# argumentcomputer/multi-stark

Hardware: AMD Instinct MI355X
Metric: prove_trace_rows_per_sec (higher is better)
Workload: dtype u64; 1 GPU; U32-add + byte-table lookup (benches/multi_stark.rs), 2^20 additions per proof, bench_config(): log_blowup 2, 100 queries, 10+10 PoW bits, GoldilocksBlake3Config; witness (traces + claims, 64-bit words) in pinned host memory at step start: upload, from_stage_1 on the device and read-back inside the timed region; the library narrows byte-valued traces on host threads INSIDE the step before they cro; rows_per_proof=1048832, proof_bytes=1100053, parallelism=single GPU

## Files before the change

### multi-stark_amd/csrc/b3_quad.h

```cpp
#pragma once
#include "b3_dev.h"

namespace msamd {

namespace b3q {
constexpr unsigned char S[7][16] = {{0, 1, 2, 3, 4, 5, 6, 7, 8, 9, 10, 11, 12, 13, 14, 15},
                                    {2, 6, 3, 10, 7, 0, 4, 13, 1, 11, 12, 5, 9, 14, 15, 8},
                                    {3, 4, 10, 12, 13, 2, 7, 14, 6, 5, 9, 0, 11, 15, 8, 1},
                                    {10, 7, 12, 9, 14, 3, 13, 15, 4, 0, 11, 2, 5, 8, 1, 6},
                                    {12, 13, 9, 11, 15, 10, 14, 8, 7, 2, 5, 3, 0, 1, 6, 4},
                                    {9, 14, 11, 5, 8, 12, 15, 1, 13, 3, 0, 10, 2, 6, 4, 7},
                                    {11, 15, 5, 0, 1, 9, 8, 6, 14, 10, 2, 12, 3, 4, 7, 13}};
constexpr u32 packed(int r, int k) {
  u32 p = 0;
  for (int c = 0; c < 4; c++) {
    int pos = (k < 2 ? 2 * c + k : 8 + 2 * c + (k - 2));
    p |= (u32)S[r][pos] << (4 * c);
  }
  return p;
}
__device__ __forceinline__ u32 qperm(u32 x, int ctrl) {
#if !defined(__HIP_DEVICE_COMPILE__)
  return x;
#else
// ... 39 lines not shown
#pragma unroll
  for (int r = 0; r < 7; r++) {
    B3Q_G(mw[r][0], mw[r][1])
    b = b3q::qperm(b, 0x39);
    cc = b3q::qperm(cc, 0x4E);
    d = b3q::qperm(d, 0x93);
    B3Q_G(mw[r][2], mw[r][3])
    b = b3q::qperm(b, 0x93);
    cc = b3q::qperm(cc, 0x4E);
    d = b3q::qperm(d, 0x39);
  }
  h_lo = a ^ cc;
  h_hi = b ^ d;
}

__device__ __forceinline__ void b3_quad_compress_cv(const u32* msg, u32 block_len, u32 flags, u32& lo, u32& hi) {
  const u32 c = threadIdx.x & 3;
  const u32 sh4 = 4 * c;
  u32 mw[7][4];
#pragma unroll
  for (int r = 0; r < 7; r++) {
#pragma unroll
    for (int k = 0; k < 4; k++) mw[r][k] = msg[(b3q::packed(r, k) >> sh4) & 15u];
  }
  u32 a = lo, b = hi;
  u32 cc = c == 0 ? B3_IV0 : c == 1 ? B3_IV1 : c == 2 ? B3_IV2 : B3_IV3;
  u32 d = c == 2 ? block_len : c == 3 ? flags : 0u;
#pragma unroll
  for (int r = 0; r < 7; r++) {
    B3Q_G(mw[r][0], mw[r][1])
    b = b3q::qperm(b, 0x39);
    cc = b3q::qperm(cc, 0x4E);
    d = b3q::qperm(d, 0x93);
    B3Q_G(mw[r][2], mw[r][3])
    b = b3q::qperm(b, 0x93);
    cc = b3q::qperm(cc, 0x4E);
    d = b3q::qperm(d, 0x39);
  }
  lo = a ^ cc;
  hi = b ^ d;
}

// ... 9 lines not shown
```

### multi-stark_amd/csrc/hash.hip

```cpp
#include <algorithm>
#include <cstdlib>
#include <cstring>

#include "b3_dev.h"
#include "b3_quad.h"
#include "outer_dev.h"
#include "challenge_dev.h"
#include "fri_dev.h"
#include "msamd.h"
#include "tree_dev.h"

namespace msamd {

namespace {

struct RowIter {
  const MatRef* g;
  size_t H, row;
  unsigned mi;
  u32 c;
  const u64* cur;
  u32 w;
  size_t stride;
  __device__ __forceinline__ void init() {
// ... 511 lines not shown
    }
  }
  if (CH) {
    challenger_round<1024>(cs, sh, p.fc.pow_bits);
    if (t < 8) {
      p.fc.state[t] = cs.st[t];
      p.fc.rec->root[t] = sh[t];
    }
    if (t == 0) {
      p.fc.rec->witness = cs.wit;
      p.fc.rec->beta = cs.beta;
    }
  }
}

__device__ __forceinline__ u32 stream_byte(const uint8_t* __restrict__ prefix, size_t pl, const u64* __restrict__ words, size_t p) {
  if (p < pl) return prefix[p];
  size_t q = p - pl;
  return (u32)((words[q >> 3] >> (8 * (q & 7))) & 0xff);
}

__global__ __launch_bounds__(256) void chunk_cv_k(const uint8_t* __restrict__ prefix, size_t pl, const u64* __restrict__ words,
                                                  size_t len, size_t nchunks, size_t c0, size_t c1, Digest* out) {
  size_t ch = c0 + blockIdx.x * size_t(blockDim.x) + threadIdx.x;
  if (ch >= c1) return;
  size_t off = ch * 1024;
  size_t clen = len - off < 1024 ? len - off : 1024;
  u32 nblocks = clen == 0 ? 1 : (u32)((clen + 63) / 64);
  u32 cv[8];
  b3_iv(cv);
  const bool single = nchunks == 1;
  for (u32 b = 0; b < nblocks; b++) {
    u32 m[16];
    size_t boff = off + size_t(b) * 64;
    u32 bl = (u32)(clen - size_t(b) * 64 < 64 ? clen - size_t(b) * 64 : 64);
    if (bl == 64 && boff >= pl) {
      size_t q = boff - pl;
      const u64* w = words + (q >> 3);
      unsigned s = (unsigned)(q & 7) * 8;
      u64 cur = w[0];
#pragma unroll
      for (int k = 0; k < 8; k++) {
        u64 x;
        if (s == 0) {
          x = cur;
          if (k < 7) cur = w[k + 1];
        } else {
          u64 nxt = w[k + 1];
          x = (cur >> s) | (nxt << (64 - s));
          cur = nxt;
        }
        m[2 * k] = (u32)x;
        m[2 * k + 1] = (u32)(x >> 32);
      }
    } else {
#pragma unroll
      for (int i = 0; i < 16; i++) {
        u32 wv = 0;
        for (int k = 0; k < 4; k++) {
          u32 idx = 4 * i + k;
          u32 byte = idx < bl ? stream_byte(prefix, pl, words, boff + idx) : 0;
          wv |= byte << (8 * k);
        }
        m[i] = wv;
      }
    }
    u32 flags = (b == 0 ? B3_CHUNK_START : 0) | (b == nblocks - 1 ? (B3_CHUNK_END | (single ? B3_ROOT : 0)) : 0);
    b3_compress(cv, m, ch, bl, flags);
  }
  store_digest(out + ch, cv);
}

__global__ __launch_bounds__(64) void chunk_cv_prefix_k(const uint8_t* __restrict__ prefix, size_t pl, const u64* __restrict__ words,
                                                        size_t len, size_t nchunks, size_t c0, Digest* out) {
  __shared__ u32 sh[256];
  const size_t ch = c0 + blockIdx.x;
  const size_t off = ch * 1024;
  const size_t clen = len - off < 1024 ? len - off : 1024;
  for (u32 i = threadIdx.x; i < 256; i += 64) {
    u32 wv = 0;
#pragma unroll
    for (u32 k = 0; k < 4; k++) {
      const u32 idx = 4 * i + k;
      const u32 byte = idx < clen ? stream_byte(prefix, pl, words, off + idx) : 0;
      wv |= byte << (8 * k);
    }
    sh[i] = wv;
  }
  __syncthreads();
  if (threadIdx.x != 0) return;
  const u32 nblocks = clen == 0 ? 1 : (u32)((clen + 63) / 64);
  u32 cv[8];
  b3_iv(cv);
  const bool single = nchunks == 1;
  for (u32 b = 0; b < nblocks; b++) {
    u32 m[16];
#pragma unroll
    for (int i = 0; i < 16; i++) m[i] = sh[16 * b + i];
    const u32 bl = (u32)(clen - size_t(b) * 64 < 64 ? clen - size_t(b) * 64 : 64);
    const u32 flags = (b == 0 ? B3_CHUNK_START : 0) | (b == nblocks - 1 ? (B3_CHUNK_END | (single ? B3_ROOT : 0)) : 0);
    b3_compress(cv, m, ch, bl, flags);
  }
  store_digest(out + ch, cv);
}

__global__ __launch_bounds__(256) void cv_level_k(const Digest* __restrict__ prev, Digest* __restrict__ next, size_t n_prev,
                                                  u32 root_flag) {
  size_t n_next = (n_prev + 1) / 2;
  size_t i = blockIdx.x * size_t(blockDim.x) + threadIdx.x;
  if (i >= n_next) return;
  u32 l[8];
  load_digest(prev + 2 * i, l);
  if (2 * i + 1 < n_prev) {
    u32 r[8], o[8];
    load_digest(prev + 2 * i + 1, r);
    parent_cv(l, r, root_flag, o);
    store_digest(next + i, o);
  } else {
    store_digest(next + i, l);
  }
}

__global__ __launch_bounds__(1024) void cv_tail_k(const Digest* __restrict__ prev, Digest* __restrict__ out, u32 n, Digest* __restrict__ sib_out = nullptr) {
  __shared__ __attribute__((aligned(16))) u32 sh[2048 * 8];
  const u32 t = threadIdx.x;
  for (u32 i = t; i < n; i += 1024) {
    u32 d[8];
    load_digest(prev + i, d);
    lds_store_digest(sh, i, d);
  }
  __syncthreads();
  const u32 quad = t >> 2, c = t & 3;
  while (n > 1) {
    const u32 nn = (n + 1) / 2;
    const u32 flags = B3_PARENT | (n == 2 ? (u32)B3_ROOT : 0u);
    if (sib_out) {
      if (t < 8) reinterpret_cast<u32*>(sib_out)[t] = sh[8 + t];
      sib_out++;
    }
    u32 lo[4], hi[4];
#pragma unroll
    for (int ps = 0; ps < 4; ps++) {
      const u32 q = quad + 256 * ps;
      if (q < nn) {
        if (2 * q + 1 < n) {
          b3_quad_compress_iv<false>(sh + 16 * q, 64, flags, lo[ps], hi[ps]);
        } else {
          lo[ps] = sh[16 * q + c];
          hi[ps] = sh[16 * q + 4 + c];
        }
      }
    }
    __syncthreads();
#pragma unroll
    for (int ps = 0; ps < 4; ps++) {
      const u32 q = quad + 256 * ps;
      if (q < nn) {
        sh[8 * q + c] = lo[ps];
        sh[8 * q + 4 + c] = hi[ps];
      }
    }
    __syncthreads();
    n = nn;
  }
  if (t < 8) reinterpret_cast<u32*>(out)[t] = sh[t];
}

}

void merkle_alloc(Ctx& ctx, DTree& t, size_t maxh) {
  t.layer_off.clear();
  t.layer_len.clear();
  size_t tot = 0;
  for (size_t l = maxh;; l >>= 1) {
    t.layer_off.push_back(tot);
    t.layer_len.push_back(l);
    tot += l;
    if (l == 1) break;
  }
  t.digests = DBuf<Digest>(ctx, tot);
// ... 252 lines not shown
  HIP_CHECK(hipGetLastError());
}

std::vector<Digest> merkle_cap(Ctx& ctx, const DTree& t) {
  size_t cl = t.cap_layer();
  std::vector<Digest> cap(t.layer_len[cl]);
  ctx.d2h(cap.data(), t.base() + t.layer_off[cl], cap.size() * sizeof(Digest));
  return cap;
}

size_t blake3_num_chunks(size_t prefix_len, size_t nwords) {
  size_t len = prefix_len + 8 * nwords;
  return len == 0 ? 1 : (len + 1023) / 1024;
}

void blake3_chunk_cvs(Ctx& ctx, const uint8_t* d_prefix, size_t prefix_len, const u64* d_words, size_t nwords, size_t c0, size_t c1,
                      Digest* cvs) {
  const size_t len = prefix_len + 8 * nwords, nchunks = blake3_num_chunks(prefix_len, nwords);
  if (c1 > nchunks) c1 = nchunks;
  if (c0 >= c1) return;
  const size_t pc = std::min(c1, (prefix_len + 1023) / 1024);
  if (c0 < pc) {
    hipLaunchKernelGGL(chunk_cv_prefix_k, dim3((unsigned)(pc - c0)), dim3(64), 0, ctx.stream, d_prefix, prefix_len, d_words, len, nchunks, c0, cvs);
    c0 = pc;
  }
  if (c0 < c1)
    hipLaunchKernelGGL(chunk_cv_k, dim3((unsigned)((c1 - c0 + 255) / 256)), dim3(256), 0, ctx.stream, d_prefix, prefix_len, d_words, len,
                       nchunks, c0, c1, cvs);
  HIP_CHECK(hipGetLastError());
}

struct ClaimsRootArgs {
  const uint8_t* prefix;
  const u64* words;
  size_t pl, len;
  const u32* cap;
  u32 cap_off, cap_bytes;
  const Digest* sib[32];
  u32 nchunks;
  Digest* out;
  ChallengeBG* bg;
  u32* state_out;
};
__global__ __launch_bounds__(64) void claims_root_k(ClaimsRootArgs a) {
  __shared__ u32 sh[256];
  __shared__ u32 pm[16];
  const u32 t = threadIdx.x, c = t & 3;
  const u32 clen = a.len < 1024 ? (u32)a.len : 1024u;
  for (u32 i = t; i < 256; i += 64) {
    u32 wv = 0;
#pragma unroll
    for (u32 k = 0; k < 4; k++) {
      const u32 idx = 4 * i + k;
      u32 byte = 0;
      if (idx < clen) {
        if (idx >= a.cap_off && idx - a.cap_off < a.cap_bytes) {
          const u32 q = idx - a.cap_off;
          byte = (a.cap[q >> 2] >> (8 * (q & 3))) & 0xff;
        } else {
          byte = stream_byte(a.prefix, a.pl, a.words, idx);
        }
      }
      wv |= byte << (8 * k);
    }
    sh[i] = wv;
  }
  __syncthreads();
  u32 lo = c == 0 ? B3_IV0 : c == 1 ? B3_IV1 : c == 2 ? B3_IV2 : B3_IV3;
  u32 hi = c == 0 ? B3_IV4 : c == 1 ? B3_IV5 : c == 2 ? B3_IV6 : B3_IV7;
  const u32 nblocks = (clen + 63) / 64;
  for (u32 b = 0; b < nblocks; b++) {
    const u32 bl = clen - 64 * b < 64 ? clen - 64 * b : 64;
    const u32 flags = (b == 0 ? (u32)B3_CHUNK_START : 0u) | (b == nblocks - 1 ? (u32)B3_CHUNK_END : 0u);
    b3_quad_compress_cv(sh + 16 * b, bl, flags, lo, hi);
  }
  for (u32 l = 0; (1u << l) < a.nchunks; l++) {
    if (t < 4) {
      pm[c] = lo;
      pm[4 + c] = hi;
    }
    if (t >= 8 && t < 16) pm[t] = reinterpret_cast<const u32*>(a.sib[l])[t - 8];
    __syncthreads();
    const bool last = (2u << l) >= a.nchunks;
    b3_quad_compress_iv<false>(pm, 64, B3_PARENT | (last ? (u32)B3_ROOT : 0u), lo, hi);
    __syncthreads();
  }
  if (t < 4) {
    u32* o = reinterpret_cast<u32*>(a.out);
    o[c] = lo;
    o[4 + c] = hi;
    pm[c] = lo;
    pm[4 + c] = hi;
  }
  if (a.bg) {
    __syncthreads();
    outer_beta_gamma_step(pm, a.bg, a.state_out);
  }
}

static const Digest* blake3_cv_tree(Ctx& ctx, Digest* cvs, size_t nchunks, DBuf<Digest>& scratch, Digest* out_dev) {
  scratch = DBuf<Digest>(ctx, (nchunks + 1) / 2);
  Digest* cur = cvs;
  Digest* nxt = scratch.p;
  size_t n = nchunks;
  while (n > 1) {
    if (n <= 2048) {
      hipLaunchKernelGGL(cv_tail_k, dim3(1), dim3(1024), 0, ctx.stream, (const Digest*)cur, nxt, (u32)n);
      std::swap(cur, nxt);
      break;
    }
    size_t nn = (n + 1) / 2;
    hipLaunchKernelGGL(cv_level_k, dim3((unsigned)((nn + 255) / 256)), dim3(256), 0, ctx.stream, cur, nxt, n,
                       n == 2 ? (u32)B3_ROOT : 0u);
    std::swap(cur, nxt);
    n = nn;
  }
  HIP_CHECK(hipGetLastError());
  if (out_dev) HIP_CHECK(hipMemcpyAsync(out_dev, cur, sizeof(Digest), hipMemcpyDeviceToDevice, ctx.stream));
  return cur;
}
Digest blake3_from_cvs(Ctx& ctx, Digest* cvs, size_t nchunks) {
  DBuf<Digest> b;
  const Digest* cur = blake3_cv_tree(ctx, cvs, nchunks, b, nullptr);
  Digest out;
  ctx.d2h(&out, cur, sizeof(Digest));
  return out;
}
void blake3_from_cvs_async(Ctx& ctx, Digest* cvs, size_t nchunks, Digest* out_dev) {
  DBuf<Digest> b;
  (void)blake3_cv_tree(ctx, cvs, nchunks, b, out_dev);
}

void blake3_late_chunk0_prepare(Ctx& ctx, const Digest* cvs, size_t nchunks, LateChunk0& lc) {
  if (nchunks < 2 || nchunks > (size_t(1) << 30)) throw std::runtime_error("blake3_late_chunk0: chunk count out of range");
  lc.levels = DBuf<Digest>(ctx, nchunks + 64);
  lc.sib.clear();
  const Digest* cur = cvs;
  Digest* nxt = lc.levels.p;
  size_t n = nchunks;
  while (n > 1) {
    if (n <= 2048) {
      Digest* tail_sib = nxt + 1;
      size_t m = n;
      while (m > 1) {
        lc.sib.push_back(tail_sib++);
        m = (m + 1) / 2;
      }
      hipLaunchKernelGGL(cv_tail_k, dim3(1), dim3(1024), 0, ctx.stream, cur, nxt, (u32)n, nxt + 1);
      break;
    }
    lc.sib.push_back(cur + 1);
    const size_t nn = (n + 1) / 2;
    hipLaunchKernelGGL(cv_level_k, dim3((unsigned)((nn + 255) / 256)), dim3(256), 0, ctx.stream, cur, nxt, n, 0u);
    cur = nxt;
    nxt += nn;
    n = nn;
  }
  HIP_CHECK(hipGetLastError());
  if (lc.sib.size() > 32) throw std::runtime_error("blake3_late_chunk0: too many levels");
}
void blake3_late_chunk0_finish(Ctx& ctx, const uint8_t* d_prefix, size_t prefix_len, const u64* d_words, size_t nwords, const Digest* d_cap,
                               size_t cap_off, size_t ncap, const LateChunk0& lc, size_t nchunks, Digest* out_dev, ChallengeBG* d_bg,
                               u32* d_state12) {
  if (prefix_len > 1024 || cap_off + 32 * ncap > prefix_len) throw std::runtime_error("blake3_late_chunk0: the prefix must lie inside chunk 0");
  ClaimsRootArgs a;
  memset(&a, 0, sizeof(a));
  a.prefix = d_prefix;
  a.words = d_words;
  a.pl = prefix_len;
  a.len = prefix_len + 8 * nwords;
  a.cap = reinterpret_cast<const u32*>(d_cap);
  a.cap_off = (u32)cap_off;
  a.cap_bytes = (u32)(32 * ncap);
  unsigned levels = 0;
  while ((size_t(1) << levels) < nchunks) levels++;
  if (lc.sib.size() != levels) throw std::runtime_error("blake3_late_chunk0: level count mismatch");
  for (unsigned l = 0; l < levels; l++) a.sib[l] = lc.sib[l];
  a.nchunks = (u32)nchunks;
  a.out = out_dev;
  a.bg = d_bg;
  a.state_out = d_state12;
  hipLaunchKernelGGL(claims_root_k, dim3(1), dim3(64), 0, ctx.stream, a);
  HIP_CHECK(hipGetLastError());
}

Digest blake3_device(Ctx& ctx, const uint8_t* d_prefix, size_t prefix_len, const u64* d_words, size_t nwords) {
  const size_t nchunks = blake3_num_chunks(prefix_len, nwords);
  DBuf<Digest> a(ctx, nchunks);
  blake3_chunk_cvs(ctx, d_prefix, prefix_len, d_words, nwords, 0, nchunks, a.p);
  return blake3_from_cvs(ctx, a.p, nchunks);
}

}
```

### multi-stark_amd/csrc/msamd.h

```cpp
#pragma once
#include <hip/hip_runtime.h>

#include <cstdint>
#include <cstring>
#include <map>
#include <mutex>
#include <stdexcept>
#include <string>
#include <vector>

#include "gl_dev.h"

namespace msamd {

#define HIP_CHECK(expr)                                                                                   \
  do {                                                                                                    \
    hipError_t _e = (expr);                                                                               \
    if (_e != hipSuccess)                                                                                 \
      throw std::runtime_error(std::string("HIP error: ") + hipGetErrorString(_e) + " at " + __FILE__ + ":" + \
                               std::to_string(__LINE__));                                                 \
  } while (0)

static constexpr unsigned TW_LOG = 28;
static constexpr unsigned TW_HALF = 14;
// ... 208 lines not shown
  std::vector<size_t> layer_off, layer_len;
  unsigned cap_height = 0;
  size_t max_height() const { return layer_len.empty() ? 0 : layer_len[0]; }
  size_t cap_layer() const {
    size_t L = layer_len.size();
    size_t ch = cap_height < L - 1 ? cap_height : L - 1;
    return L - 1 - ch;
  }
};
void merkle_build(Ctx& ctx, DTree& t);
void merkle_alloc(Ctx& ctx, DTree& t, size_t max_height);
struct FriChallenge;
void merkle_compress_plain(Ctx& ctx, DTree& t, const FriChallenge* fc = nullptr);
std::vector<Digest> merkle_cap(Ctx& ctx, const DTree& t);
void merkle_tree_top(Ctx& ctx, const Digest* d_roots, size_t n, Digest* d_out);
Digest blake3_device(Ctx& ctx, const uint8_t* d_prefix, size_t prefix_len, const u64* d_words, size_t nwords);
size_t blake3_num_chunks(size_t prefix_len, size_t nwords);
void blake3_chunk_cvs(Ctx& ctx, const uint8_t* d_prefix, size_t prefix_len, const u64* d_words, size_t nwords, size_t c0, size_t c1,
                      Digest* cvs);
Digest blake3_from_cvs(Ctx& ctx, Digest* cvs, size_t nchunks);
void blake3_from_cvs_async(Ctx& ctx, Digest* cvs, size_t nchunks, Digest* out_dev);
struct ChallengeBG;
struct LateChunk0 {
  DBuf<Digest> levels;
  std::vector<const Digest*> sib;
  void reset() {
    levels.reset();
    sib.clear();
  }
};
void blake3_late_chunk0_prepare(Ctx& ctx, const Digest* cvs, size_t nchunks, LateChunk0& lc);
void blake3_late_chunk0_finish(Ctx& ctx, const uint8_t* d_prefix, size_t prefix_len, const u64* d_words, size_t nwords, const Digest* d_cap,
                               size_t cap_off, size_t ncap, const LateChunk0& lc, size_t nchunks, Digest* out_dev,
                               ChallengeBG* d_bg = nullptr ,
                               u32* d_state12 = nullptr);

struct JitKernel;
struct DLookups {
  size_t height = 0, num_lookups = 0, args_width = 0;
  DBuf<u64> mult, args;
  DBuf<uint32_t> arg_offsets;
};
E2 stage2_build(Ctx& ctx, const DLookups& lk, E2 beta, E2 gamma, u64* out_colmajor_bitrev, const JitKernel* jit = nullptr);
void stage2_build_async(Ctx& ctx, const DLookups& lk, E2 beta, E2 gamma, u64* out_colmajor_bitrev, E2* total_dev,
                        const JitKernel* jit = nullptr);
struct ChallengeBG;
DBuf<ChallengeBG> challenge_bg_upload(Ctx& ctx, E2 beta, E2 gamma);
// ... 170 lines not shown
```

### multi-stark_amd/csrc/prover.hip

```cpp
#include <algorithm>
#include <chrono>
#include <cstdio>
#include <cstdlib>

#include <sys/resource.h>
#include <unistd.h>

#include <atomic>
#include <condition_variable>
#include <functional>
#include <mutex>
#include <thread>

#include "host.h"
#include "ingest.h"
#include "lookup_params.h"
#include "open_plan.h"
#include "quotient_params.h"

namespace msamd {

namespace {
void load_block(const uint8_t* p, size_t len, u32 w[16]) {
  uint8_t buf[64];
// ... 1755 lines not shown
void observe_claims(Ctx& ctx, Challenger& ch, HWitness& wit) {
  const size_t n_claims = wit.claim_offsets.size() - 1;
  const size_t claim_elems = wit.claim_data.size();
  const size_t claim_words = 1 + n_claims + claim_elems;
  if (claim_words <= 8192) {
    ch.observe((u64)n_claims);
    for (size_t i = 0; i < n_claims; i++) {
      size_t a = wit.claim_offsets[i], b = wit.claim_offsets[i + 1];
      ch.observe((u64)(b - a));
      for (size_t k = a; k < b; k++) ch.observe(wit.claim_data[k]);
    }
    return;
  }
  DBuf<uint8_t> d_prefix(ctx, ch.input.size());
  ctx.h2d(d_prefix.p, ch.input.data(), ch.input.size());
  DBuf<u64> d_words(ctx, claim_words);
  claims_transcript_words(ctx, wit.d_claim_data.p, wit.d_claim_offsets.p, n_claims, claim_elems, d_words.p);
  Digest d = blake3_device(ctx, d_prefix.p, ch.input.size(), d_words.p, claim_words);
  ch.flush_with(d);
}

std::vector<uint8_t> prove(HSystem& sys, HWitness& wit, StageMs* times) {
  Ctx& ctx = *sys.ctx;
  HIP_CHECK(hipSetDevice(ctx.device));
  const Params& prm = sys.params;
  const unsigned lb = (unsigned)prm.log_blowup;
  const size_t C = sys.circuits.size();
  if (wit.sys != &sys || wit.heights.size() != C) throw std::runtime_error("witness does not belong to this system");
  if (wit.has_remote) throw std::runtime_error("this witness lacks traces that another rank computes: use ms_prove_sharded");
  double t_begin = now_ms(), t0;
  g_probes.start();
  auto lap = [&](int slot) {
    if (times) {
// ... 50 lines not shown
  } side_session{ctx};
  auto fork_side = [&]() {
    if (use_side && !ctx.side_forked) ctx.side_fork();
  };

  const size_t n_claims = wit.claim_offsets.size() - 1;
  const size_t claim_elems = wit.claim_data.size();
  const size_t claim_words = 1 + n_claims + claim_elems;
  const bool device_claims = claim_words > 8192;
  const bool early_claims = device_claims && ctx.side_enabled;
  size_t max_lde_log = 0;
  for (unsigned ld : log_degrees) max_lde_log = std::max<size_t>(max_lde_log, ld + lb);
  const size_t ncap = size_t(1) << std::min<size_t>((size_t)prm.cap_height, max_lde_log);
  std::vector<Digest> s1_cap;
  size_t cap_off = 0, prefix_chunks = 0, nchunks = 0;
  DBuf<u64> d_words;
  DBuf<Digest> d_cvs;
  const bool dev_outer = device_claims && outer_fits(ncap, NA) && !getenv("MSAMD_HOST_TRANSCRIPT");
  OuterDev od;
  DBuf<ChallengeBG> d_bg;
  if (device_claims) {
    s1_cap.assign(ncap, Digest());
    if (sys.has_pre) ch.observe_cap(sys.pre_commit);
    cap_off = ch.input.size();
    ch.observe_cap(s1_cap);
    for (unsigned ld : log_degrees) ch.observe(ld);
    nchunks = blake3_num_chunks(ch.input.size(), claim_words);
    prefix_chunks = std::min(nchunks, (ch.input.size() + 1023) / 1024);
  }
  const bool late_chunk0 = device_claims && prefix_chunks == 1 && nchunks >= 2 && !getenv("MSAMD_OLD_CLAIMS_TREE");
  LateChunk0 late0;
  DBuf<uint8_t> d_prefix;
  auto claims_chunks = [&]() {
    up.wait_claims();
    d_words = DBuf<u64>(ctx, claim_words);
    claims_transcript_words(ctx, wit.d_claim_data.p, wit.d_claim_offsets.p, n_claims, claim_elems, d_words.p);
    d_cvs = DBuf<Digest>(ctx, nchunks);
    blake3_chunk_cvs(ctx, nullptr, ch.input.size(), d_words.p, claim_words, prefix_chunks, nchunks, d_cvs.p);
    d_prefix = DBuf<uint8_t>(ctx, ch.input.size());
    ctx.h2d(d_prefix.p, ch.input.data(), ch.input.size());
    if (late_chunk0) blake3_late_chunk0_prepare(ctx, d_cvs.p, nchunks, late0);
  };

  t0 = now_ms();
  RoctxRange phase("stark/stage1_commit");
  PcsData s1;
  {
    std::vector<DMat> ldes(NA);
    up.wait_traces();
    fork_side();
    for (size_t pos : order) {
      const size_t ci = aidx[pos];
      SideScope sc(ctx, on_side[pos]);
// ... 22 lines not shown
      for (size_t k = a; k < b; k++) ch.observe(wit.claim_data[k]);
    }
  } else {
    lap(0);
    const size_t cl = s1.tree.cap_layer();
    if (s1.tree.layer_len[cl] != ncap) throw std::runtime_error("stage-1 cap size differs from the transcript's placeholder");
    const Digest* d_cap = s1.tree.base() + s1.tree.layer_off[cl];
    if (!early_claims) claims_chunks();
    ctx.side_join();
    od.digest = DBuf<Digest>(ctx, 1);
    if (dev_outer) {
      od.state = DBuf<u32>(ctx, 28);
      d_bg = DBuf<ChallengeBG>(ctx, 1);
    }
    if (late_chunk0) {
      blake3_late_chunk0_finish(ctx, d_prefix.p, ch.input.size(), d_words.p, claim_words, d_cap, cap_off, ncap, late0, nchunks, od.digest.p,
                                dev_outer ? d_bg.p : nullptr, dev_outer ? od.state.p : nullptr);
    } else {
      HIP_CHECK(hipMemcpyAsync(d_prefix.p + cap_off, d_cap, ncap * sizeof(Digest), hipMemcpyDeviceToDevice, ctx.stream));
      blake3_chunk_cvs(ctx, d_prefix.p, ch.input.size(), d_words.p, claim_words, 0, prefix_chunks, d_cvs.p);
      blake3_from_cvs_async(ctx, d_cvs.p, nchunks, od.digest.p);
    }
    ctx.d2h_queue(s1_cap.data(), d_cap, ncap * sizeof(Digest));
    if (dev_outer) {
      if (!late_chunk0) outer_beta_gamma(ctx, od.digest.p, d_bg.p, od.state.p);
      ctx.d2h_queue(&od.h_digest, od.digest.p, sizeof(Digest));
      ctx.d2h_queue(od.h_bg, d_bg.p, 2 * sizeof(E2));
      g_probes.mark("claims digest + beta/gamma queued");
    } else {
      Digest d;
      ctx.d2h(&d, od.digest.p, sizeof(Digest));
      g_probes.mark("sync 1 (cap + claims digest)");
      ch.flush_with(d);
    }
    d_words.reset();
    d_cvs.reset();
    late0.reset();
    d_prefix.reset();
  }
  E2 beta = e2(0), gamma = e2(0), alpha = e2(0), zeta = e2(0);
  if (!dev_outer) {
    tx_beta_gamma(ch, beta, gamma);
    d_bg = challenge_bg_upload(ctx, beta, gamma);
  }
  DBuf<E2> d_tot(ctx, NA + 1);
  std::vector<E2> h_tot(NA + 1);
  const bool claims_on_device = n_claims > 256 || dev_outer;
  const bool claims_beside = claims_on_device && ctx.side_enabled && !getenv("MSAMD_CLAIMS_ACC_MAIN");
  auto claims_sum_launch = [&]() {
    if (claims_beside && !ctx.side_forked) ctx.side_fork();
// ... 254 lines not shown
```

Measured before the change: 158.7 million rows/s.

## Hash claims transcript in place with quad-lane BLAKE3 chunks and single-kernel CV tree

```diff
diff --git a/multi-stark_amd/csrc/b3_quad.h b/multi-stark_amd/csrc/b3_quad.h
--- a/multi-stark_amd/csrc/b3_quad.h
+++ b/multi-stark_amd/csrc/b3_quad.h
@@ -77,7 +77,7 @@
   h_hi = b ^ d;
 }
 
-__device__ __forceinline__ void b3_quad_compress_cv(const u32* msg, u32 block_len, u32 flags, u32& lo, u32& hi) {
+__device__ __forceinline__ void b3_quad_compress_cv(const u32* msg, u32 block_len, u32 flags, u32& lo, u32& hi, u64 counter = 0) {
   const u32 c = threadIdx.x & 3;
   const u32 sh4 = 4 * c;
   u32 mw[7][4];
@@ -88,7 +88,7 @@
   }
   u32 a = lo, b = hi;
   u32 cc = c == 0 ? B3_IV0 : c == 1 ? B3_IV1 : c == 2 ? B3_IV2 : B3_IV3;
-  u32 d = c == 2 ? block_len : c == 3 ? flags : 0u;
+  u32 d = c == 0 ? (u32)counter : c == 1 ? (u32)(counter >> 32) : c == 2 ? block_len : flags;
 #pragma unroll
   for (int r = 0; r < 7; r++) {
     B3Q_G(mw[r][0], mw[r][1])
diff --git a/multi-stark_amd/csrc/hash.hip b/multi-stark_amd/csrc/hash.hip
--- a/multi-stark_amd/csrc/hash.hip
+++ b/multi-stark_amd/csrc/hash.hip
@@ -549,98 +549,136 @@
   }
 }
 
-__device__ __forceinline__ u32 stream_byte(const uint8_t* __restrict__ prefix, size_t pl, const u64* __restrict__ words, size_t p) {
-  if (p < pl) return prefix[p];
-  size_t q = p - pl;
-  return (u32)((words[q >> 3] >> (8 * (q & 7))) & 0xff);
-}
-
-__global__ __launch_bounds__(256) void chunk_cv_k(const uint8_t* __restrict__ prefix, size_t pl, const u64* __restrict__ words,
-                                                  size_t len, size_t nchunks, size_t c0, size_t c1, Digest* out) {
-  size_t ch = c0 + blockIdx.x * size_t(blockDim.x) + threadIdx.x;
-  if (ch >= c1) return;
-  size_t off = ch * 1024;
-  size_t clen = len - off < 1024 ? len - off : 1024;
-  u32 nblocks = clen == 0 ? 1 : (u32)((clen + 63) / 64);
-  u32 cv[8];
-  b3_iv(cv);
+struct StreamArgs {
+  const uint8_t* prefix;
+  size_t pl, len;
+  StreamWords src;
+  const u32* cap;
+  u32 cap_off, cap_bytes;
+};
+
+constexpr u32 CHUNKS_PER_WAVE = 16;
+constexpr u32 CHUNK_LDS = 1024 + 16;
+__device__ __forceinline__ u32 chunk_lds_off(u32 o) { return o + (o >> 10) * 16; }
+
+__device__ __forceinline__ void stage_put(uint8_t* shb, long off, long lim, u64 v) {
+  if ((off & 3) == 0) {
+    if (off >= 0 && off < lim) *reinterpret_cast<u32*>(shb + chunk_lds_off((u32)off)) = (u32)v;
+    if (off + 4 >= 0 && off + 4 < lim) *reinterpret_cast<u32*>(shb + chunk_lds_off((u32)(off + 4))) = (u32)(v >> 32);
+  } else if ((off & 1) == 0) {
+#pragma unroll
+    for (int k = 0; k < 4; k++) {
+      const long o = off + 2 * k;
+      if (o >= 0 && o < lim) *reinterpret_cast<uint16_t*>(shb + chunk_lds_off((u32)o)) = (uint16_t)(v >> (16 * k));
+    }
+  } else {
+#pragma unroll
+    for (int k = 0; k < 8; k++) {
+      const long o = off + k;
+      if (o >= 0 && o < lim) shb[chunk_lds_off((u32)o)] = (uint8_t)(v >> (8 * k));
+    }
+  }
+}
+
+__device__ __forceinline__ void stage_stream(uint8_t* shb, const StreamArgs& a, size_t b0, u32 nb) {
+  const u32 lane = threadIdx.x;
+  const size_t bend = b0 + nb < a.len ? b0 + nb : a.len;
+  const long lim = bend > b0 ? (long)(bend - b0) : 0;
+  if (lim < (long)nb) {
+    for (u32 o = ((u32)lim & ~3u) + 4 * lane; o < nb; o += 256) *reinterpret_cast<u32*>(shb + chunk_lds_off(o)) = 0u;
+    __syncthreads();
+  }
+  const size_t pend = bend < a.pl ? bend : a.pl;
+  for (size_t p = b0 + lane; p < pend; p += 64) {
+    u32 byte = a.prefix[p];
+    if (a.cap && p >= a.cap_off && p - a.cap_off < a.cap_bytes) {
+      const u32 q = (u32)(p - a.cap_off);
+      byte = (a.cap[q >> 2] >> (8 * (q & 3))) & 0xff;
+    }
+    shb[chunk_lds_off((u32)(p - b0))] = (uint8_t)byte;
+  }
+  if (bend > a.pl) {
+    const size_t j_lo = b0 > a.pl ? (b0 - a.pl) >> 3 : 0, j_hi = (bend - a.pl + 7) >> 3;
+    const long d0 = (long)a.pl - (long)b0;
+    if (a.src.words) {
+      for (size_t j = j_lo + lane; j < j_hi; j += 64) stage_put(shb, d0 + 8 * (long)j, lim, a.src.words[j]);
+    } else {
+      const u64* __restrict__ offs = a.src.offs;
+      const u64* __restrict__ data = a.src.data;
+      const size_t n = a.src.n;
+      if (j_lo == 0 && lane == 0) stage_put(shb, d0, lim, (u64)n);
+      size_t i0 = 0;
+      if (j_lo > 1 && n > 0) {
+        size_t lo = 0, hi = n - 1;
+        while (lo < hi) {
+          const size_t step = (hi - lo + 63) / 64;
+          size_t probe = lo + (lane + 1) * step;
+          if (probe > hi) probe = hi;
+          const bool ok = 1 + probe + (size_t)offs[probe] <= j_lo;
+          const u32 cnt = (u32)__popcll(__ballot(ok));
+          const size_t hi_new = cnt < 64 ? lo + (cnt + 1) * step - 1 : hi;
+          if (cnt) lo = lo + cnt * step < hi ? lo + cnt * step : hi;
+          if (hi_new < hi) hi = hi_new;
+        }
+        i0 = lo;
+      }
+      size_t i = i0 + lane;
+      u64 o_cur = i < n ? offs[i] : 0, o_nxt = i < n ? offs[i + 1] : 0;
+      for (;;) {
+        const size_t i2 = i + 64;
+        const u64 p_cur = i2 < n ? offs[i2] : 0, p_nxt = i2 < n ? offs[i2 + 1] : 0;
+        const size_t o = (size_t)o_cur, s = 1 + i + o;
+        const bool past = i >= n || s >= j_hi;
+        if (!past) {
+          const size_t clen = (size_t)o_nxt - o;
+          if (s >= j_lo) stage_put(shb, d0 + 8 * (long)s, lim, (u64)clen);
+          const size_t k0 = s + 1 < j_lo ? j_lo - (s + 1) : 0;
+          const size_t k1 = clen < j_hi - (s + 1) ? clen : j_hi - (s + 1);
+          for (size_t k = k0; k < k1; k += 4) {
+            u64 v[4];
+#pragma unroll
+            for (int u = 0; u < 4; u++) v[u] = k + u < k1 ? data[o + k + u] : 0;
+#pragma unroll
+            for (int u = 0; u < 4; u++)
+              if (k + u < k1) stage_put(shb, d0 + 8 * (long)(s + 1 + k + u), lim, v[u]);
+          }
+        }
+        if (__any(past)) break;
+        i = i2;
+        o_cur = p_cur;
+        o_nxt = p_nxt;
+      }
+    }
+  }
+  __syncthreads();
+}
+
+__global__ __launch_bounds__(64) void chunk_cv_k(StreamArgs a, size_t nchunks, size_t c0, size_t c1, Digest* out) {
+  __shared__ __attribute__((aligned(16))) uint8_t shb[CHUNKS_PER_WAVE * CHUNK_LDS];
+  const size_t cb = c0 + size_t(blockIdx.x) * CHUNKS_PER_WAVE;
+  if (cb >= c1) return;
+  const u32 cnt = c1 - cb < CHUNKS_PER_WAVE ? (u32)(c1 - cb) : CHUNKS_PER_WAVE;
+  stage_stream(shb, a, cb * 1024, cnt * 1024);
+  const u32 q = threadIdx.x >> 2, c = threadIdx.x & 3;
+  if (q >= cnt) return;
+  const size_t ch = cb + q, off = ch * 1024;
+  const u32 clen = a.len <= off ? 0u : a.len - off < 1024 ? (u32)(a.len - off) : 1024u;
+  const u32 nblocks = clen == 0 ? 1 : (clen + 63) / 64;
+  const u32* m = reinterpret_cast<const u32*>(shb + q * CHUNK_LDS);
+  u32 lo = c == 0 ? B3_IV0 : c == 1 ? B3_IV1 : c == 2 ? B3_IV2 : B3_IV3;
+  u32 hi = c == 0 ? B3_IV4 : c == 1 ? B3_IV5 : c == 2 ? B3_IV6 : B3_IV7;
   const bool single = nchunks == 1;
   for (u32 b = 0; b < nblocks; b++) {
-    u32 m[16];
-    size_t boff = off + size_t(b) * 64;
-    u32 bl = (u32)(clen - size_t(b) * 64 < 64 ? clen - size_t(b) * 64 : 64);
-    if (bl == 64 && boff >= pl) {
-      size_t q = boff - pl;
-      const u64* w = words + (q >> 3);
-      unsigned s = (unsigned)(q & 7) * 8;
-      u64 cur = w[0];
-#pragma unroll
-      for (int k = 0; k < 8; k++) {
-        u64 x;
-        if (s == 0) {
-          x = cur;
-          if (k < 7) cur = w[k + 1];
-        } else {
-          u64 nxt = w[k + 1];
-          x = (cur >> s) | (nxt << (64 - s));
-          cur = nxt;
-        }
-        m[2 * k] = (u32)x;
-        m[2 * k + 1] = (u32)(x >> 32);
-      }
-    } else {
-#pragma unroll
-      for (int i = 0; i < 16; i++) {
-        u32 wv = 0;
-        for (int k = 0; k < 4; k++) {
-          u32 idx = 4 * i + k;
-          u32 byte = idx < bl ? stream_byte(prefix, pl, words, boff + idx) : 0;
-          wv |= byte << (8 * k);
-        }
-        m[i] = wv;
-      }
-    }
-    u32 flags = (b == 0 ? B3_CHUNK_START : 0) | (b == nblocks - 1 ? (B3_CHUNK_END | (single ? B3_ROOT : 0)) : 0);
-    b3_compress(cv, m, ch, bl, flags);
-  }
-  store_digest(out + ch, cv);
-}
-
-__global__ __launch_bounds__(64) void chunk_cv_prefix_k(const uint8_t* __restrict__ prefix, size_t pl, const u64* __restrict__ words,
-                                                        size_t len, size_t nchunks, size_t c0, Digest* out) {
-  __shared__ u32 sh[256];
-  const size_t ch = c0 + blockIdx.x;
-  const size_t off = ch * 1024;
-  const size_t clen = len - off < 1024 ? len - off : 1024;
-  for (u32 i = threadIdx.x; i < 256; i += 64) {
-    u32 wv = 0;
-#pragma unroll
-    for (u32 k = 0; k < 4; k++) {
-      const u32 idx = 4 * i + k;
-      const u32 byte = idx < clen ? stream_byte(prefix, pl, words, off + idx) : 0;
-      wv |= byte << (8 * k);
-    }
-    sh[i] = wv;
-  }
-  __syncthreads();
-  if (threadIdx.x != 0) return;
-  const u32 nblocks = clen == 0 ? 1 : (u32)((clen + 63) / 64);
-  u32 cv[8];
-  b3_iv(cv);
-  const bool single = nchunks == 1;
-  for (u32 b = 0; b < nblocks; b++) {
-    u32 m[16];
-#pragma unroll
-    for (int i = 0; i < 16; i++) m[i] = sh[16 * b + i];
-    const u32 bl = (u32)(clen - size_t(b) * 64 < 64 ? clen - size_t(b) * 64 : 64);
-    const u32 flags = (b == 0 ? B3_CHUNK_START : 0) | (b == nblocks - 1 ? (B3_CHUNK_END | (single ? B3_ROOT : 0)) : 0);
-    b3_compress(cv, m, ch, bl, flags);
-  }
-  store_digest(out + ch, cv);
-}
-
-__global__ __launch_bounds__(256) void cv_level_k(const Digest* __restrict__ prev, Digest* __restrict__ next, size_t n_prev,
-                                                  u32 root_flag) {
+    const u32 bl = clen - 64 * b < 64 ? clen - 64 * b : 64;
+    const u32 flags = (b == 0 ? (u32)B3_CHUNK_START : 0u) | (b == nblocks - 1 ? (u32)B3_CHUNK_END | (single ? (u32)B3_ROOT : 0u) : 0u);
+    b3_quad_compress_cv(m + 16 * b, bl, flags, lo, hi, (u64)ch);
+  }
+  u32* o = reinterpret_cast<u32*>(out + ch);
+  o[c] = lo;
+  o[4 + c] = hi;
+}
+
+__global__ __launch_bounds__(256) void cv_level_k(const Digest* __restrict__ prev, Digest* __restrict__ next, size_t n_prev) {
   size_t n_next = (n_prev + 1) / 2;
   size_t i = blockIdx.x * size_t(blockDim.x) + threadIdx.x;
   if (i >= n_next) return;
@@ -649,56 +687,98 @@
   if (2 * i + 1 < n_prev) {
     u32 r[8], o[8];
     load_digest(prev + 2 * i + 1, r);
-    parent_cv(l, r, root_flag, o);
+    parent_cv(l, r, 0u, o);
     store_digest(next + i, o);
   } else {
     store_digest(next + i, l);
   }
 }
 
-__global__ __launch_bounds__(1024) void cv_tail_k(const Digest* __restrict__ prev, Digest* __restrict__ out, u32 n, Digest* __restrict__ sib_out = nullptr) {
-  __shared__ __attribute__((aligned(16))) u32 sh[2048 * 8];
+constexpr u32 CV_SUB = 2048, CV_SUB_LEVELS = 11;
+__device__ __forceinline__ void cv_reduce(u32* sh, u32 n, bool root_here, Digest* sib) {
   const u32 t = threadIdx.x;
-  for (u32 i = t; i < n; i += 1024) {
-    u32 d[8];
-    load_digest(prev + i, d);
-    lds_store_digest(sh, i, d);
-  }
-  __syncthreads();
-  const u32 quad = t >> 2, c = t & 3;
   while (n > 1) {
     const u32 nn = (n + 1) / 2;
-    const u32 flags = B3_PARENT | (n == 2 ? (u32)B3_ROOT : 0u);
-    if (sib_out) {
-      if (t < 8) reinterpret_cast<u32*>(sib_out)[t] = sh[8 + t];
-      sib_out++;
-    }
-    u32 lo[4], hi[4];
-#pragma unroll
-    for (int ps = 0; ps < 4; ps++) {
-      const u32 q = quad + 256 * ps;
+    const u32 root = root_here && n == 2 ? (u32)B3_ROOT : 0u;
+    if (sib) {
+      if (t < 8) reinterpret_cast<u32*>(sib)[t] = sh[8 + t];
+      sib++;
+    }
+    if (nn >= 128) {
+      u32 d[8];
+      const bool act = t < nn;
+      if (act) {
+        lds_load_digest(sh, 2 * t, d);
+        if (2 * t + 1 < n) {
+          u32 l[8], r[8];
+#pragma unroll
+          for (int k = 0; k < 8; k++) l[k] = d[k];
+          lds_load_digest(sh, 2 * t + 1, r);
+          parent_cv(l, r, root, d);
+        }
+      }
+      __syncthreads();
+      if (act) lds_store_digest(sh, t, d);
+      __syncthreads();
+    } else {
+      const u32 q = t >> 2, c = t & 3;
+      u32 lo = 0, hi = 0;
       if (q < nn) {
         if (2 * q + 1 < n) {
-          b3_quad_compress_iv<false>(sh + 16 * q, 64, flags, lo[ps], hi[ps]);
+          b3_quad_compress_iv<false>(sh + 16 * q, 64, B3_PARENT | root, lo, hi);
         } else {
-          lo[ps] = sh[16 * q + c];
-          hi[ps] = sh[16 * q + 4 + c];
+          lo = sh[16 * q + c];
+          hi = sh[16 * q + 4 + c];
         }
       }
-    }
+      __syncthreads();
+      if (q < nn) {
+        sh[8 * q + c] = lo;
+        sh[8 * q + 4 + c] = hi;
+      }
+      __syncthreads();
+    }
+    n = nn;
+  }
+}
+
+struct CvTreeArgs {
+  const Digest* cvs;
+  u32 n;
+  Digest* roots;
+  u32* counter;
+  Digest* out;
+  Digest* sib;
+};
+__global__ __launch_bounds__(1024) void cv_tree_k(CvTreeArgs a) {
+  __shared__ __attribute__((aligned(16))) u32 sh[CV_SUB * 8];
+  __shared__ u32 s_last;
+  const u32 t = threadIdx.x, nb = gridDim.x, b = blockIdx.x;
+  const u32 m = a.n - CV_SUB * b < CV_SUB ? a.n - CV_SUB * b : CV_SUB;
+  for (u32 i = t; i < m; i += 1024) {
+    u32 d[8];
+    load_digest(a.cvs + size_t(b) * CV_SUB + i, d);
+    lds_store_digest(sh, i, d);
+  }
+  __syncthreads();
+  cv_reduce(sh, m, nb == 1, b == 0 ? a.sib : nullptr);
+  if (nb > 1) {
+    if (t < 8) __hip_atomic_store(reinterpret_cast<u32*>(a.roots + b) + t, sh[t], __ATOMIC_RELAXED, __HIP_MEMORY_SCOPE_AGENT);
+    asm volatile("s_waitcnt vmcnt(0)" ::: "memory");
     __syncthreads();
-#pragma unroll
-    for (int ps = 0; ps < 4; ps++) {
-      const u32 q = quad + 256 * ps;
-      if (q < nn) {
-        sh[8 * q + c] = lo[ps];
-        sh[8 * q + 4 + c] = hi[ps];
-      }
+    if (t == 0) {
+      const u32 ticket = __hip_atomic_fetch_add(a.counter, 1u, __ATOMIC_RELAXED, __HIP_MEMORY_SCOPE_AGENT);
+      s_last = ticket == nb - 1 ? 1u : 0u;
     }
     __syncthreads();
-    n = nn;
-  }
-  if (t < 8) reinterpret_cast<u32*>(out)[t] = sh[t];
+    if (!s_last) return;
+    const u32* rw = reinterpret_cast<const u32*>(a.roots);
+    for (u32 i = t; i < nb * 8; i += 1024) sh[i] = __hip_atomic_load(rw + i, __ATOMIC_RELAXED, __HIP_MEMORY_SCOPE_AGENT);
+    if (t == 0) __hip_atomic_store(a.counter, 0u, __ATOMIC_RELAXED, __HIP_MEMORY_SCOPE_AGENT);
+    __syncthreads();
+    cv_reduce(sh, nb, true, a.sib ? a.sib + CV_SUB_LEVELS : nullptr);
+  }
+  if (t < 8) reinterpret_cast<u32*>(a.out)[t] = sh[t];
 }
 
 }
@@ -981,28 +1061,23 @@
   return len == 0 ? 1 : (len + 1023) / 1024;
 }
 
-void blake3_chunk_cvs(Ctx& ctx, const uint8_t* d_prefix, size_t prefix_len, const u64* d_words, size_t nwords, size_t c0, size_t c1,
+void blake3_chunk_cvs(Ctx& ctx, const uint8_t* d_prefix, size_t prefix_len, const StreamWords& src, size_t nwords, size_t c0, size_t c1,
                       Digest* cvs) {
-  const size_t len = prefix_len + 8 * nwords, nchunks = blake3_num_chunks(prefix_len, nwords);
+  const size_t nchunks = blake3_num_chunks(prefix_len, nwords);
   if (c1 > nchunks) c1 = nchunks;
   if (c0 >= c1) return;
-  const size_t pc = std::min(c1, (prefix_len + 1023) / 1024);
-  if (c0 < pc) {
-    hipLaunchKernelGGL(chunk_cv_prefix_k, dim3((unsigned)(pc - c0)), dim3(64), 0, ctx.stream, d_prefix, prefix_len, d_words, len, nchunks, c0, cvs);
-    c0 = pc;
-  }
-  if (c0 < c1)
-    hipLaunchKernelGGL(chunk_cv_k, dim3((unsigned)((c1 - c0 + 255) / 256)), dim3(256), 0, ctx.stream, d_prefix, prefix_len, d_words, len,
-                       nchunks, c0, c1, cvs);
+  StreamArgs a{};
+  a.prefix = d_prefix;
+  a.pl = prefix_len;
+  a.len = prefix_len + 8 * nwords;
+  a.src = src;
+  hipLaunchKernelGGL(chunk_cv_k, dim3((unsigned)((c1 - c0 + CHUNKS_PER_WAVE - 1) / CHUNKS_PER_WAVE)), dim3(64), 0, ctx.stream, a, nchunks, c0, c1,
+                     cvs);
   HIP_CHECK(hipGetLastError());
 }
 
 struct ClaimsRootArgs {
-  const uint8_t* prefix;
-  const u64* words;
-  size_t pl, len;
-  const u32* cap;
-  u32 cap_off, cap_bytes;
+  StreamArgs s;
   const Digest* sib[32];
   u32 nchunks;
   Digest* out;
@@ -1010,29 +1085,14 @@
   u32* state_out;
 };
 __global__ __launch_bounds__(64) void claims_root_k(ClaimsRootArgs a) {
-  __shared__ u32 sh[256];
+  __shared__ __attribute__((aligned(16))) uint8_t shb[CHUNK_LDS];
+  __shared__ u32 sibs[32 * 8];
   __shared__ u32 pm[16];
+  const u32* sh = reinterpret_cast<const u32*>(shb);
   const u32 t = threadIdx.x, c = t & 3;
-  const u32 clen = a.len < 1024 ? (u32)a.len : 1024u;
-  for (u32 i = t; i < 256; i += 64) {
-    u32 wv = 0;
-#pragma unroll
-    for (u32 k = 0; k < 4; k++) {
-      const u32 idx = 4 * i + k;
-      u32 byte = 0;
-      if (idx < clen) {
-        if (idx >= a.cap_off && idx - a.cap_off < a.cap_bytes) {
-          const u32 q = idx - a.cap_off;
-          byte = (a.cap[q >> 2] >> (8 * (q & 3))) & 0xff;
-        } else {
-          byte = stream_byte(a.prefix, a.pl, a.words, idx);
-        }
-      }
-      wv |= byte << (8 * k);
-    }
-    sh[i] = wv;
-  }
-  __syncthreads();
+  const u32 clen = a.s.len < 1024 ? (u32)a.s.len : 1024u;
+  for (u32 i = t; (1u << (i >> 3)) < a.nchunks; i += 64) sibs[i] = reinterpret_cast<const u32*>(a.sib[i >> 3])[i & 7];
+  stage_stream(shb, a.s, 0, 1024);
   u32 lo = c == 0 ? B3_IV0 : c == 1 ? B3_IV1 : c == 2 ? B3_IV2 : B3_IV3;
   u32 hi = c == 0 ? B3_IV4 : c == 1 ? B3_IV5 : c == 2 ? B3_IV6 : B3_IV7;
   const u32 nblocks = (clen + 63) / 64;
@@ -1046,7 +1106,7 @@
       pm[c] = lo;
       pm[4 + c] = hi;
     }
-    if (t >= 8 && t < 16) pm[t] = reinterpret_cast<const u32*>(a.sib[l])[t - 8];
+    if (t >= 8 && t < 16) pm[t] = sibs[8 * l + t - 8];
     __syncthreads();
     const bool last = (2u << l) >= a.nchunks;
     b3_quad_compress_iv<false>(pm, 64, B3_PARENT | (last ? (u32)B3_ROOT : 0u), lo, hi);
@@ -1065,26 +1125,44 @@
   }
 }
 
+static constexpr size_t CV_TREE_MAX = size_t(CV_SUB) * CV_SUB;
+static size_t cv_tree_scratch(size_t n) { return (n > CV_TREE_MAX ? n + 64 : 0) + CV_SUB + 32; }
+static void cv_tree_launch(Ctx& ctx, const Digest* cvs, size_t n, Digest* scratch, Digest* out, std::vector<const Digest*>* sibs) {
+  const Digest* cur = cvs;
+  Digest* nxt = scratch;
+  while (n > CV_TREE_MAX) {
+    if (sibs) sibs->push_back(cur + 1);
+    const size_t nn = (n + 1) / 2;
+    hipLaunchKernelGGL(cv_level_k, dim3((unsigned)((nn + 255) / 256)), dim3(256), 0, ctx.stream, cur, nxt, n);
+    cur = nxt;
+    nxt += nn;
+    n = nn;
+  }
+  CvTreeArgs a{};
+  a.cvs = cur;
+  a.n = (u32)n;
+  a.roots = nxt;
+  a.counter = tree_counter_slot(ctx) + 1;
+  a.out = out;
+  if (sibs) {
+    a.sib = nxt + CV_SUB;
+    Digest* s = a.sib;
+    for (size_t m = n; m > 1; m = (m + 1) / 2) sibs->push_back(s++);
+  }
+  hipLaunchKernelGGL(cv_tree_k, dim3((unsigned)((n + CV_SUB - 1) / CV_SUB)), dim3(1024), 0, ctx.stream, a);
+  HIP_CHECK(hipGetLastError());
+}
+
 static const Digest* blake3_cv_tree(Ctx& ctx, Digest* cvs, size_t nchunks, DBuf<Digest>& scratch, Digest* out_dev) {
-  scratch = DBuf<Digest>(ctx, (nchunks + 1) / 2);
-  Digest* cur = cvs;
-  Digest* nxt = scratch.p;
-  size_t n = nchunks;
-  while (n > 1) {
-    if (n <= 2048) {
-      hipLaunchKernelGGL(cv_tail_k, dim3(1), dim3(1024), 0, ctx.stream, (const Digest*)cur, nxt, (u32)n);
-      std::swap(cur, nxt);
-      break;
-    }
-    size_t nn = (n + 1) / 2;
-    hipLaunchKernelGGL(cv_level_k, dim3((unsigned)((nn + 255) / 256)), dim3(256), 0, ctx.stream, cur, nxt, n,
-                       n == 2 ? (u32)B3_ROOT : 0u);
-    std::swap(cur, nxt);
-    n = nn;
-  }
-  HIP_CHECK(hipGetLastError());
-  if (out_dev) HIP_CHECK(hipMemcpyAsync(out_dev, cur, sizeof(Digest), hipMemcpyDeviceToDevice, ctx.stream));
-  return cur;
+  if (nchunks == 1) {
+    if (out_dev) HIP_CHECK(hipMemcpyAsync(out_dev, cvs, sizeof(Digest), hipMemcpyDeviceToDevice, ctx.stream));
+    return out_dev ? out_dev : cvs;
+  }
+  const size_t ns = cv_tree_scratch(nchunks);
+  scratch = DBuf<Digest>(ctx, ns + 1);
+  Digest* out = out_dev ? out_dev : scratch.p + ns;
+  cv_tree_launch(ctx, cvs, nchunks, scratch.p, out, nullptr);
+  return out;
 }
 Digest blake3_from_cvs(Ctx& ctx, Digest* cvs, size_t nchunks) {
   DBuf<Digest> b;
@@ -1100,45 +1178,24 @@
 
 void blake3_late_chunk0_prepare(Ctx& ctx, const Digest* cvs, size_t nchunks, LateChunk0& lc) {
   if (nchunks < 2 || nchunks > (size_t(1) << 30)) throw std::runtime_error("blake3_late_chunk0: chunk count out of range");
-  lc.levels = DBuf<Digest>(ctx, nchunks + 64);
+  const size_t ns = cv_tree_scratch(nchunks);
+  lc.levels = DBuf<Digest>(ctx, ns + 1);
   lc.sib.clear();
-  const Digest* cur = cvs;
-  Digest* nxt = lc.levels.p;
-  size_t n = nchunks;
-  while (n > 1) {
-    if (n <= 2048) {
-      Digest* tail_sib = nxt + 1;
-      size_t m = n;
-      while (m > 1) {
-        lc.sib.push_back(tail_sib++);
-        m = (m + 1) / 2;
-      }
-      hipLaunchKernelGGL(cv_tail_k, dim3(1), dim3(1024), 0, ctx.stream, cur, nxt, (u32)n, nxt + 1);
-      break;
-    }
-    lc.sib.push_back(cur + 1);
-    const size_t nn = (n + 1) / 2;
-    hipLaunchKernelGGL(cv_level_k, dim3((unsigned)((nn + 255) / 256)), dim3(256), 0, ctx.stream, cur, nxt, n, 0u);
-    cur = nxt;
-    nxt += nn;
-    n = nn;
-  }
-  HIP_CHECK(hipGetLastError());
+  cv_tree_launch(ctx, cvs, nchunks, lc.levels.p, lc.levels.p + ns , &lc.sib);
   if (lc.sib.size() > 32) throw std::runtime_error("blake3_late_chunk0: too many levels");
 }
-void blake3_late_chunk0_finish(Ctx& ctx, const uint8_t* d_prefix, size_t prefix_len, const u64* d_words, size_t nwords, const Digest* d_cap,
+void blake3_late_chunk0_finish(Ctx& ctx, const uint8_t* d_prefix, size_t prefix_len, const StreamWords& src, size_t nwords, const Digest* d_cap,
                                size_t cap_off, size_t ncap, const LateChunk0& lc, size_t nchunks, Digest* out_dev, ChallengeBG* d_bg,
                                u32* d_state12) {
   if (prefix_len > 1024 || cap_off + 32 * ncap > prefix_len) throw std::runtime_error("blake3_late_chunk0: the prefix must lie inside chunk 0");
-  ClaimsRootArgs a;
-  memset(&a, 0, sizeof(a));
-  a.prefix = d_prefix;
-  a.words = d_words;
-  a.pl = prefix_len;
-  a.len = prefix_len + 8 * nwords;
-  a.cap = reinterpret_cast<const u32*>(d_cap);
-  a.cap_off = (u32)cap_off;
-  a.cap_bytes = (u32)(32 * ncap);
+  ClaimsRootArgs a{};
+  a.s.prefix = d_prefix;
+  a.s.src = src;
+  a.s.pl = prefix_len;
+  a.s.len = prefix_len + 8 * nwords;
+  a.s.cap = reinterpret_cast<const u32*>(d_cap);
+  a.s.cap_off = (u32)cap_off;
+  a.s.cap_bytes = (u32)(32 * ncap);
   unsigned levels = 0;
   while ((size_t(1) << levels) < nchunks) levels++;
   if (lc.sib.size() != levels) throw std::runtime_error("blake3_late_chunk0: level count mismatch");
@@ -1151,10 +1208,11 @@
   HIP_CHECK(hipGetLastError());
 }
 
-Digest blake3_device(Ctx& ctx, const uint8_t* d_prefix, size_t prefix_len, const u64* d_words, size_t nwords) {
+
+Digest blake3_device(Ctx& ctx, const uint8_t* d_prefix, size_t prefix_len, const StreamWords& src, size_t nwords) {
   const size_t nchunks = blake3_num_chunks(prefix_len, nwords);
   DBuf<Digest> a(ctx, nchunks);
-  blake3_chunk_cvs(ctx, d_prefix, prefix_len, d_words, nwords, 0, nchunks, a.p);
+  blake3_chunk_cvs(ctx, d_prefix, prefix_len, src, nwords, 0, nchunks, a.p);
   return blake3_from_cvs(ctx, a.p, nchunks);
 }
 
diff --git a/multi-stark_amd/csrc/msamd.h b/multi-stark_amd/csrc/msamd.h
--- a/multi-stark_amd/csrc/msamd.h
+++ b/multi-stark_amd/csrc/msamd.h
@@ -246,9 +246,24 @@
 void merkle_compress_plain(Ctx& ctx, DTree& t, const FriChallenge* fc = nullptr);
 std::vector<Digest> merkle_cap(Ctx& ctx, const DTree& t);
 void merkle_tree_top(Ctx& ctx, const Digest* d_roots, size_t n, Digest* d_out);
-Digest blake3_device(Ctx& ctx, const uint8_t* d_prefix, size_t prefix_len, const u64* d_words, size_t nwords);
+struct StreamWords {
+  const u64* words = nullptr;
+  const u64* offs = nullptr;
+  const u64* data = nullptr;
+  size_t n = 0;
+  StreamWords() = default;
+  StreamWords(const u64* w) : words(w) {}
+  static StreamWords claims(const u64* d_claim_offsets, const u64* d_claim_data, size_t n_claims) {
+    StreamWords s;
+    s.offs = d_claim_offsets;
+    s.data = d_claim_data;
+    s.n = n_claims;
+    return s;
+  }
+};
+Digest blake3_device(Ctx& ctx, const uint8_t* d_prefix, size_t prefix_len, const StreamWords& src, size_t nwords);
 size_t blake3_num_chunks(size_t prefix_len, size_t nwords);
-void blake3_chunk_cvs(Ctx& ctx, const uint8_t* d_prefix, size_t prefix_len, const u64* d_words, size_t nwords, size_t c0, size_t c1,
+void blake3_chunk_cvs(Ctx& ctx, const uint8_t* d_prefix, size_t prefix_len, const StreamWords& src, size_t nwords, size_t c0, size_t c1,
                       Digest* cvs);
 Digest blake3_from_cvs(Ctx& ctx, Digest* cvs, size_t nchunks);
 void blake3_from_cvs_async(Ctx& ctx, Digest* cvs, size_t nchunks, Digest* out_dev);
@@ -262,7 +277,7 @@
   }
 };
 void blake3_late_chunk0_prepare(Ctx& ctx, const Digest* cvs, size_t nchunks, LateChunk0& lc);
-void blake3_late_chunk0_finish(Ctx& ctx, const uint8_t* d_prefix, size_t prefix_len, const u64* d_words, size_t nwords, const Digest* d_cap,
+void blake3_late_chunk0_finish(Ctx& ctx, const uint8_t* d_prefix, size_t prefix_len, const StreamWords& src, size_t nwords, const Digest* d_cap,
                                size_t cap_off, size_t ncap, const LateChunk0& lc, size_t nchunks, Digest* out_dev,
                                ChallengeBG* d_bg = nullptr ,
                                u32* d_state12 = nullptr);
diff --git a/multi-stark_amd/csrc/prover.hip b/multi-stark_amd/csrc/prover.hip
--- a/multi-stark_amd/csrc/prover.hip
+++ b/multi-stark_amd/csrc/prover.hip
@@ -1793,9 +1793,7 @@
   }
   DBuf<uint8_t> d_prefix(ctx, ch.input.size());
   ctx.h2d(d_prefix.p, ch.input.data(), ch.input.size());
-  DBuf<u64> d_words(ctx, claim_words);
-  claims_transcript_words(ctx, wit.d_claim_data.p, wit.d_claim_offsets.p, n_claims, claim_elems, d_words.p);
-  Digest d = blake3_device(ctx, d_prefix.p, ch.input.size(), d_words.p, claim_words);
+  Digest d = blake3_device(ctx, d_prefix.p, ch.input.size(), StreamWords::claims(wit.d_claim_offsets.p, wit.d_claim_data.p, n_claims), claim_words);
   ch.flush_with(d);
 }
 
@@ -1876,7 +1874,6 @@
   const size_t ncap = size_t(1) << std::min<size_t>((size_t)prm.cap_height, max_lde_log);
   std::vector<Digest> s1_cap;
   size_t cap_off = 0, prefix_chunks = 0, nchunks = 0;
-  DBuf<u64> d_words;
   DBuf<Digest> d_cvs;
   const bool dev_outer = device_claims && outer_fits(ncap, NA) && !getenv("MSAMD_HOST_TRANSCRIPT");
   OuterDev od;
@@ -1893,12 +1890,11 @@
   const bool late_chunk0 = device_claims && prefix_chunks == 1 && nchunks >= 2 && !getenv("MSAMD_OLD_CLAIMS_TREE");
   LateChunk0 late0;
   DBuf<uint8_t> d_prefix;
+  auto claims_in_place = [&]() { return StreamWords::claims(wit.d_claim_offsets.p, wit.d_claim_data.p, n_claims); };
   auto claims_chunks = [&]() {
     up.wait_claims();
-    d_words = DBuf<u64>(ctx, claim_words);
-    claims_transcript_words(ctx, wit.d_claim_data.p, wit.d_claim_offsets.p, n_claims, claim_elems, d_words.p);
     d_cvs = DBuf<Digest>(ctx, nchunks);
-    blake3_chunk_cvs(ctx, nullptr, ch.input.size(), d_words.p, claim_words, prefix_chunks, nchunks, d_cvs.p);
+    blake3_chunk_cvs(ctx, nullptr, ch.input.size(), claims_in_place(), claim_words, prefix_chunks, nchunks, d_cvs.p);
     d_prefix = DBuf<uint8_t>(ctx, ch.input.size());
     ctx.h2d(d_prefix.p, ch.input.data(), ch.input.size());
     if (late_chunk0) blake3_late_chunk0_prepare(ctx, d_cvs.p, nchunks, late0);
@@ -1951,11 +1947,11 @@
       d_bg = DBuf<ChallengeBG>(ctx, 1);
     }
     if (late_chunk0) {
-      blake3_late_chunk0_finish(ctx, d_prefix.p, ch.input.size(), d_words.p, claim_words, d_cap, cap_off, ncap, late0, nchunks, od.digest.p,
+      blake3_late_chunk0_finish(ctx, d_prefix.p, ch.input.size(), claims_in_place(), claim_words, d_cap, cap_off, ncap, late0, nchunks, od.digest.p,
                                 dev_outer ? d_bg.p : nullptr, dev_outer ? od.state.p : nullptr);
     } else {
       HIP_CHECK(hipMemcpyAsync(d_prefix.p + cap_off, d_cap, ncap * sizeof(Digest), hipMemcpyDeviceToDevice, ctx.stream));
-      blake3_chunk_cvs(ctx, d_prefix.p, ch.input.size(), d_words.p, claim_words, 0, prefix_chunks, d_cvs.p);
+      blake3_chunk_cvs(ctx, d_prefix.p, ch.input.size(), claims_in_place(), claim_words, 0, prefix_chunks, d_cvs.p);
       blake3_from_cvs_async(ctx, d_cvs.p, nchunks, od.digest.p);
     }
     ctx.d2h_queue(s1_cap.data(), d_cap, ncap * sizeof(Digest));
@@ -1970,7 +1966,6 @@
       g_probes.mark("sync 1 (cap + claims digest)");
       ch.flush_with(d);
     }
-    d_words.reset();
     d_cvs.reset();
     late0.reset();
     d_prefix.reset();
```

Result: no change. 161.3 million rows/s, median of 4 (+1.6%).
